# HansiZeng/scaling-retriever

Hardware: AMD Instinct MI355X
Metric: MSMARCO-Dev queries/sec end-to-end (query encode + dense brute-force top-1000) (higher is better)
Workload: dtype f32

## Files before the change

### include/sr_hip.h

```cpp
#ifndef SR_HIP_H
#define SR_HIP_H
#include <stdint.h>
#ifdef __cplusplus
extern "C" {
#endif

#define SR_OK 0
#define SR_ERR_INVALID 1
#define SR_ERR_HIP 2
#define SR_ERR_NOMEM 3
#define SR_ERR_UNSUPPORTED 4

#define SR_DTYPE_F32 0
#define SR_DTYPE_BF16 1
#define SR_DTYPE_F16 2

typedef void* sr_stream;

const char* sr_last_error(void);
int sr_version(void);
int sr_max_topk(void);

typedef struct sr_dense_index sr_dense_index;

// ... 193 lines not shown
                   sr_stream stream);
int sr_encode_rows(sr_model* m, const int64_t* d_input_ids, const int64_t* d_attention_mask, int32_t B, int32_t L,
                   const int32_t* d_row_shift, int32_t mode, int32_t fp32, float* d_out_sparse, float* d_out_dense,
                   sr_stream stream);
int sr_model_last_hidden(sr_model* m, float* d_out, int64_t capacity_rows, int64_t* n_tokens, sr_stream stream);
int sr_model_destroy(sr_model* m);

int sr_lora_merge(float* d_W, const float* d_A, const float* d_B, int64_t out_features,
                  int64_t in_features, int32_t r, float scale, sr_stream stream);

int sr_sparse_compact(const float* d_reps, int64_t B, int64_t V, int64_t* d_row_ptr,
                      int32_t* d_cols, float* d_vals, int64_t capacity, int64_t* h_nnz,
                      sr_stream stream);
int sr_sparse_compact_topm(const float* d_reps, int64_t B, int64_t V, int64_t max_terms,
                           int64_t* d_row_ptr, int32_t* d_cols, float* d_vals,
                           int64_t capacity, int64_t* h_nnz, sr_stream stream);

int sr_write_run_json(const char* path, int64_t nq, int64_t k, const float* h_scores, const int64_t* h_idx, const int32_t* h_counts,
                      const int64_t* h_qid_i64, const char* h_qid_bytes, const int64_t* h_qid_off, int64_t qid_width,
                      const int64_t* h_doc_i64, const char* h_doc_bytes, const int64_t* h_doc_off, int64_t doc_width,
                      int64_t n_docs, int32_t n_threads, int64_t* bytes_written);
int sr_write_run_json_part(const char* path, int32_t part, int64_t nq, int64_t k, const float* h_scores, const int64_t* h_idx,
                           const int32_t* h_counts, const int64_t* h_qid_i64, const char* h_qid_bytes, const int64_t* h_qid_off,
                           int64_t qid_width, const int64_t* h_doc_i64, const char* h_doc_bytes, const int64_t* h_doc_off,
                           int64_t doc_width, int64_t n_docs, int32_t n_threads, int64_t* bytes_written);
int64_t sr_run_writer_mapped_rounds(void);

int sr_gemm_bf16(const void* d_A, const void* d_W, int32_t M, int32_t N, int32_t K, int32_t epilogue,
                 void* d_C, const int32_t* d_seq_of, sr_stream stream);
int sr_gemm_f16_scaled(const void* d_A, const void* d_W, int32_t M, int32_t N, int32_t K, const float* d_a_scale,
                       const float* d_w_scale, float* d_C, sr_stream stream);
#define SR_READOUT_EMBED 0
#define SR_READOUT_LM_HEAD 1
#define SR_READOUT_NORM 2
#define SR_READOUT_ROPE_COS 3
#define SR_READOUT_ROPE_SIN 4
#define SR_READOUT_QKV 5
#define SR_READOUT_O 6
#define SR_READOUT_GATE_UP 7
#define SR_READOUT_DOWN 8
#define SR_READOUT_LN1 9
#define SR_READOUT_LN2 10
#define SR_READOUT_BIAS 11
#define SR_READOUT_F32 0
#define SR_READOUT_BF16 1
#define SR_READOUT_PLANES 2
#define SR_READOUT_W_INV 3
#define SR_READOUT_BF16_AS_F32 4
int sr_model_readout(sr_model* m, int32_t layer, int32_t buffer, int32_t kind, void* h_dst, int64_t capacity_bytes,
                     int64_t* n_bytes, int64_t* n_rows, int64_t* row_elems);
int sr_rows_split_f16(float* d_src, const float* d_embed, const int32_t* d_tok_id, const float* d_norm_w, float eps,
                      int32_t T, int32_t K, int32_t nseg, void* d_planes, float* d_a_inv, const float* d_gu_cmax,
                      float* d_act_sc, float* d_act_inv, sr_stream stream);
int sr_gu_cmax_f16(const void* d_wgu_planes, const float* d_wgu_inv, int32_t I, int32_t K, int32_t nseg, float* d_cmax,
                   sr_stream stream);
int sr_gemm_f16_planes(const void* d_A, const void* d_W, int32_t M, int32_t N, int32_t K, int32_t epilogue, int32_t a_nseg,
                       const float* d_a_scale, const float* d_w_scale, void* d_C, const int32_t* d_pos,
                       const float* d_rope_cos, const float* d_rope_sin, int32_t n_rope, int32_t head_dim,
                       const float* d_bias, const int32_t* d_seq_of, const float* d_out_scale, int32_t out_nseg,
                       sr_stream stream);
int sr_gemm_qkv_rope(const void* d_A, const void* d_W, int32_t M, int32_t N, int32_t K, void* d_C,
                     const int32_t* d_pos, const float* d_rope_cos, const float* d_rope_sin,
                     int32_t n_rope, int32_t head_dim, sr_stream stream);
int sr_gemm_qkv_rope_bias(const void* d_A, const void* d_W, int32_t M, int32_t N, int32_t K, void* d_C,
                          const int32_t* d_pos, const float* d_rope_cos, const float* d_rope_sin,
                          int32_t n_rope, int32_t head_dim, const float* d_bias, int32_t fp32_out, sr_stream stream);
int sr_attention_varlen(const void* d_qkv, void* d_out, const int32_t* d_cu_seqlens, const int32_t* d_pos,
                        const uint8_t* d_key_valid, const float* d_rope_cos, const float* d_rope_sin,
                        int32_t B, int32_t num_heads, int32_t num_kv_heads, int32_t head_dim, sr_stream stream);
int sr_attention_varlen_f32(const float* d_qkv, float* d_out_f32, void* d_out_planes, int32_t fp32_planes,
                            const int32_t* d_cu_seqlens, const uint8_t* d_key_valid, int32_t B, int32_t num_heads,
                            int32_t num_kv_heads, int32_t head_dim, int32_t max_seqlen, sr_stream stream);
int sr_rmsnorm_bf16(float* d_x, const float* d_embed, const int32_t* d_tok_id, const void* d_delta, const float* d_norm_w,
                    void* d_xn, float* d_xn_f32, float eps, int32_t T, int32_t H, sr_stream stream);
int sr_dense_head_pool(const float* d_x, const float* d_norm_w, const int32_t* d_cu_seqlens, const int32_t* d_pos,
                       const int32_t* d_pool_start, float eps, int32_t B, int32_t T, int32_t H, void* d_stats, float* d_out,
                       sr_stream stream);
int sr_sparse_finish(float* d_out, int64_t n, float scale, int32_t round_bf16, sr_stream stream);
int sr_encode_plan(const int64_t* d_input_ids, const int64_t* d_attention_mask, int32_t B, int32_t L, int32_t mode, int32_t vocab,
                   const int32_t* d_row_shift, int32_t* d_span_start, int32_t* d_span_len, int32_t* d_pool_start,
                   int32_t* d_row_len, int32_t* d_cu_seqlens, int32_t* d_tok_id, int32_t* d_pos, uint8_t* d_key_valid,
                   int32_t* d_seq_of, int64_t capacity, int64_t* n_tokens, sr_stream stream);
int sr_split_bf16(const float* d_src, int64_t n, void* d_p0, void* d_p1, void* d_p2, sr_stream stream);
int sr_topk_replay(const float* d_scores, const int64_t* d_ids, int64_t nq, int64_t n_stream, const int64_t* h_steps, int n_steps,
                   int k, int k2, int64_t select_over, int filter, int seg_n, int seg_group, float tau2_init, float pad_score,
                   float* d_out_scores, int64_t* d_out_ids, int32_t* d_out_counts, float* d_trace_tau, float* d_trace_tau2,
                   int32_t* d_trace_cand, int32_t* d_trace_run, uint64_t* d_trace_keys, sr_stream stream);

int sr_topk_collapse(const float* d_scores, const int64_t* d_ids, const int32_t* d_counts, int64_t nq, int64_t row_len, int exhaustive,
                     const int32_t* d_keys, int64_t n_keys, int k, float* d_out_scores, int64_t* d_out_ids, int32_t* d_out_keys,
                     int32_t* d_out_counts, int32_t* d_out_complete, sr_stream stream);

int sr_group_members_count(const int32_t* d_slot_keys, int64_t nq, int64_t kg, const int32_t* d_uniq_keys, int64_t n_groups,
                           const int64_t* d_member_indptr, const int64_t* d_member_ids, int64_t n_members,
                           const uint32_t* d_mask_words, int64_t n_masks, int64_t n_bits, const int32_t* d_query_group,
                           int64_t* d_out_indptr, int64_t* total, sr_stream stream);
int sr_group_members_fill(const int32_t* d_slot_keys, int64_t nq, int64_t kg, const int32_t* d_uniq_keys, int64_t n_groups,
                          const int64_t* d_member_indptr, const int64_t* d_member_ids, int64_t n_members,
                          const uint32_t* d_mask_words, int64_t n_masks, int64_t n_bits, const int32_t* d_query_group,
                          const int64_t* d_out_indptr, int64_t* d_out_ids, int64_t capacity, sr_stream stream);
int sr_segment_topm(const float* d_scores, const int64_t* d_ids, const int64_t* d_seg_indptr, int64_t n_segs, int m,
                    int use_threshold, float threshold, float pad_score, float* d_out_scores, int64_t* d_out_ids,
                    int32_t* d_out_counts, sr_stream stream);

#ifdef __cplusplus
}
#endif
#endif
```

### scaling_retriever_amd/_lib.py

```python
import contextlib
import ctypes
import os
import threading

_HERE = os.path.dirname(os.path.abspath(__file__))
LIB_PATH = os.environ.get("SR_HIP_LIB") or os.path.join(_HERE, "libsr_hip.so")

SR_OK, SR_ERR_INVALID, SR_ERR_HIP, SR_ERR_NOMEM, SR_ERR_UNSUPPORTED = 0, 1, 2, 3, 4
SR_DTYPE_F32, SR_DTYPE_BF16, SR_DTYPE_F16 = 0, 1, 2
SR_FUSE_RRF, SR_FUSE_MINMAX = 0, 1

c_void_p, c_int, c_int32, c_int64, c_float, c_char_p = (ctypes.c_void_p, ctypes.c_int, ctypes.c_int32,
                                                         ctypes.c_int64, ctypes.c_float, ctypes.c_char_p)


class SrModelConfig(ctypes.Structure):
    _fields_ = [
        ("vocab_size", c_int32), ("hidden_size", c_int32), ("intermediate_size", c_int32), ("num_layers", c_int32),
        ("num_heads", c_int32), ("num_kv_heads", c_int32), ("head_dim", c_int32),
        ("rms_norm_eps", c_float), ("rope_theta", c_float), ("rope_llama3", c_int32),
        ("rope_factor", c_float), ("rope_low_freq_factor", c_float), ("rope_high_freq_factor", c_float),
        ("rope_original_max_pos", c_int32), ("tie_word_embeddings", c_int32), ("has_lm_head", c_int32),
        ("max_batch_tokens", c_int32), ("max_batch_seqs", c_int32), ("fp32_planes", c_int32),
        ("attention_bias", c_int32),
# ... 59 lines not shown
                                         c_void_p, c_int64, c_int64, c_void_p, c_void_p, c_void_p, c_void_p]),
    "sr_sparse_range_count": (c_int, [c_void_p, c_void_p, c_void_p, c_void_p, c_int64, c_void_p, c_void_p, ctypes.POINTER(c_int64), c_void_p]),
    "sr_sparse_range_fill": (c_int, [c_void_p, c_void_p, c_void_p, c_void_p, c_int64, c_void_p, c_void_p, c_int64, c_int64, c_void_p,
                                     c_void_p, c_int64, c_void_p]),
    "sr_sparse_range_count_masked": (c_int, [c_void_p, c_void_p, c_void_p, c_void_p, c_int64, c_void_p, c_void_p, c_int64, c_void_p,
                                             ctypes.POINTER(c_int64), c_void_p]),
    "sr_sparse_range_fill_masked": (c_int, [c_void_p, c_void_p, c_void_p, c_void_p, c_int64, c_void_p, c_void_p, c_int64, c_void_p, c_int64,
                                            c_int64, c_void_p, c_void_p, c_int64, c_void_p]),
    "sr_sparse_range_count_grouped": (c_int, [c_void_p, c_void_p, c_void_p, c_void_p, c_int64, c_void_p, c_void_p, c_int64, c_int64, c_void_p,
                                              c_void_p, ctypes.POINTER(c_int64), c_void_p]),
    "sr_sparse_range_fill_grouped": (c_int, [c_void_p, c_void_p, c_void_p, c_void_p, c_int64, c_void_p, c_void_p, c_int64, c_int64, c_void_p,
                                             c_void_p, c_int64, c_int64, c_void_p, c_void_p, c_int64, c_void_p]),
    "sr_sparse_index_block_stats": (c_int, [c_void_p, ctypes.POINTER(c_int64), ctypes.POINTER(c_int64),
                                            ctypes.POINTER(c_int64)]),
    "sr_sparse_index_destroy": (c_int, [c_void_p]),
    "sr_sparse_index_cert_stats": (c_int, [c_void_p, ctypes.POINTER(c_int64)]),
    "sr_sparse_index_cert_debug": (c_int, [c_void_p, c_int, c_void_p, c_int64, c_void_p, c_int64,
                                           ctypes.POINTER(c_float), ctypes.POINTER(ctypes.c_int32)]),
    "sr_sparse_index_cert_readout": (c_int, [c_void_p, c_int, c_void_p, c_int64, ctypes.POINTER(c_int64)]),
    "sr_sparse_csr_expand_terms": (c_int, [c_void_p, c_int64, c_int64, c_void_p, c_void_p]),
    "sr_sparse_csr_build": (c_int, [c_void_p, c_void_p, c_void_p, c_int64, c_int64, c_int64, c_int, c_void_p, c_void_p,
                                    c_void_p, c_void_p]),
    "sr_topk_merge": (c_int, [c_void_p, c_void_p, c_int, c_int64, c_int, c_float, c_void_p, c_void_p, c_void_p]),
    "sr_topk_replay": (c_int, [c_void_p, c_void_p, c_int64, c_int64, c_void_p, c_int, c_int, c_int, c_int64, c_int, c_int, c_int, c_float,
                               c_float, c_void_p, c_void_p, c_void_p, c_void_p, c_void_p, c_void_p, c_void_p, c_void_p, c_void_p]),
    "sr_hybrid_union": (c_int, [c_void_p, c_void_p, c_int64, c_void_p, c_void_p, c_int64, c_void_p, c_int64, c_void_p, c_int64, c_int64,
                                c_void_p, c_void_p, c_void_p, c_void_p, c_int64, ctypes.POINTER(c_int64), c_void_p]),
    "sr_hybrid_rank": (c_int, [c_void_p, c_void_p, c_void_p, c_void_p, c_void_p, c_void_p, c_int64, c_float, c_float, c_int, c_void_p,
                               c_void_p, c_void_p, c_int64, c_int64, c_void_p, c_void_p, c_void_p, c_void_p, c_void_p, c_void_p]),
    "sr_rank_fuse": (c_int, [c_void_p, c_void_p, c_void_p, c_int, c_int64, c_int64, c_int, ctypes.POINTER(c_float), c_float, c_int, c_void_p,
                             c_void_p, c_void_p, c_void_p, c_void_p]),
    "sr_mmr_max_candidates": (c_int, []),
    "sr_dense_mmr": (c_int, [c_void_p, c_void_p, c_void_p, c_void_p, c_int64, c_int64, c_int, c_float, c_void_p, c_void_p, c_void_p, c_void_p,
                             c_void_p, c_void_p]),
    "sr_prf_max_entries": (c_int, []),
    "sr_sparse_feedback": (c_int, [c_void_p, c_void_p, c_void_p, c_int64, c_void_p, c_void_p, c_void_p, c_int64, c_int64, c_void_p, c_void_p,
                                   c_int64, c_int, c_int, c_float, c_float, c_float, c_int64, c_void_p, c_void_p, c_void_p, c_int64,
                                   ctypes.POINTER(c_int64), c_void_p]),
    "sr_dense_feedback": (c_int, [c_void_p, c_void_p, c_int64, c_void_p, c_void_p, c_int64, c_int, c_int, c_float, c_float, c_float, c_void_p,
                                  c_void_p]),
    "sr_topk_collapse": (c_int, [c_void_p, c_void_p, c_void_p, c_int64, c_int64, c_int, c_void_p, c_int64, c_int, c_void_p, c_void_p, c_void_p,
                                 c_void_p, c_void_p, c_void_p]),
    "sr_group_members_count": (c_int, [c_void_p, c_int64, c_int64, c_void_p, c_int64, c_void_p, c_void_p, c_int64, c_void_p, c_int64, c_int64,
                                       c_void_p, c_void_p, ctypes.POINTER(c_int64), c_void_p]),
    "sr_group_members_fill": (c_int, [c_void_p, c_int64, c_int64, c_void_p, c_int64, c_void_p, c_void_p, c_int64, c_void_p, c_int64, c_int64,
                                      c_void_p, c_void_p, c_void_p, c_int64, c_void_p]),
    "sr_segment_topm": (c_int, [c_void_p, c_void_p, c_void_p, c_int64, c_int, c_int, c_float, c_float, c_void_p, c_void_p, c_void_p,
                                c_void_p]),
    "sr_model_create": (c_int, [ctypes.POINTER(c_void_p), ctypes.POINTER(SrModelConfig)]),
    "sr_model_set_weight": (c_int, [c_void_p, c_char_p, c_void_p, c_int, c_int64, c_int64, c_void_p]),
    "sr_model_finalize": (c_int, [c_void_p]),
    "sr_model_readout": (c_int, [c_void_p, c_int32, c_int32, c_int32, c_void_p, c_int64, ctypes.POINTER(c_int64), ctypes.POINTER(c_int64),
                                 ctypes.POINTER(c_int64)]),
    "sr_model_weight_segments": (c_int, [c_void_p, ctypes.POINTER(ctypes.c_int32), c_int64, ctypes.POINTER(c_int64)]),
    "sr_model_fused_act_layers": (c_int, [c_void_p, ctypes.POINTER(ctypes.c_int32), c_int64, ctypes.POINTER(c_int64)]),
    "sr_encode_dense": (c_int, [c_void_p, c_void_p, c_void_p, c_int32, c_int32, c_void_p, c_void_p]),
    "sr_encode_sparse": (c_int, [c_void_p, c_void_p, c_void_p, c_int32, c_int32, c_void_p, c_void_p]),
    "sr_encode_dense_fp32": (c_int, [c_void_p, c_void_p, c_void_p, c_int32, c_int32, c_void_p, c_void_p]),
    "sr_encode_sparse_fp32": (c_int, [c_void_p, c_void_p, c_void_p, c_int32, c_int32, c_void_p, c_void_p]),
    "sr_encode_both": (c_int, [c_void_p, c_void_p, c_void_p, c_int32, c_int32, c_int32, c_void_p, c_void_p, c_void_p]),
    "sr_encode_rows": (c_int, [c_void_p, c_void_p, c_void_p, c_int32, c_int32, c_void_p, c_int32, c_int32, c_void_p, c_void_p, c_void_p]),
    "sr_model_last_hidden": (c_int, [c_void_p, c_void_p, c_int64, ctypes.POINTER(c_int64), c_void_p]),
    "sr_model_destroy": (c_int, [c_void_p]),
    "sr_lora_merge": (c_int, [c_void_p, c_void_p, c_void_p, c_int64, c_int64, c_int32, c_float, c_void_p]),
    "sr_run_writer_mapped_rounds": (c_int64, []),
    "sr_write_run_json": (c_int, [c_char_p, c_int64, c_int64, c_void_p, c_void_p, c_void_p, c_void_p, c_void_p, c_void_p, c_int64,
                                  c_void_p, c_void_p, c_void_p, c_int64, c_int64, c_int32, ctypes.POINTER(c_int64)]),
    "sr_write_run_json_part": (c_int, [c_char_p, c_int32, c_int64, c_int64, c_void_p, c_void_p, c_void_p, c_void_p, c_void_p, c_void_p, c_int64,
                                       c_void_p, c_void_p, c_void_p, c_int64, c_int64, c_int32, ctypes.POINTER(c_int64)]),
    "sr_gemm_bf16": (c_int, [c_void_p, c_void_p, c_int32, c_int32, c_int32, c_int32, c_void_p, c_void_p, c_void_p]),
    "sr_gemm_f16_scaled": (c_int, [c_void_p, c_void_p, c_int32, c_int32, c_int32, c_void_p, c_void_p, c_void_p, c_void_p]),
    "sr_rows_split_f16": (c_int, [c_void_p, c_void_p, c_void_p, c_void_p, c_float, c_int32, c_int32, c_int32, c_void_p, c_void_p, c_void_p,
                                  c_void_p, c_void_p, c_void_p]),
    "sr_gu_cmax_f16": (c_int, [c_void_p, c_void_p, c_int32, c_int32, c_int32, c_void_p, c_void_p]),
    "sr_gemm_f16_planes": (c_int, [c_void_p, c_void_p, c_int32, c_int32, c_int32, c_int32, c_int32, c_void_p, c_void_p, c_void_p, c_void_p,
                                   c_void_p, c_void_p, c_int32, c_int32, c_void_p, c_void_p, c_void_p, c_int32, c_void_p]),
    "sr_rmsnorm_bf16": (c_int, [c_void_p, c_void_p, c_void_p, c_void_p, c_void_p, c_void_p, c_void_p, c_float, c_int32, c_int32, c_void_p]),
    "sr_dense_head_pool": (c_int, [c_void_p, c_void_p, c_void_p, c_void_p, c_void_p, c_float, c_int32, c_int32, c_int32, c_void_p, c_void_p,
                                   c_void_p]),
    "sr_sparse_finish": (c_int, [c_void_p, c_int64, c_float, c_int32, c_void_p]),
    "sr_encode_plan": (c_int, [c_void_p, c_void_p, c_int32, c_int32, c_int32, c_int32, c_void_p, c_void_p, c_void_p, c_void_p, c_void_p,
                               c_void_p, c_void_p, c_void_p, c_void_p, c_void_p, c_int64, ctypes.POINTER(c_int64), c_void_p]),
    "sr_split_bf16": (c_int, [c_void_p, c_int64, c_void_p, c_void_p, c_void_p, c_void_p]),
    "sr_gemm_qkv_rope": (c_int, [c_void_p, c_void_p, c_int32, c_int32, c_int32, c_void_p, c_void_p, c_void_p, c_void_p,
                                 c_int32, c_int32, c_void_p]),
    "sr_gemm_qkv_rope_bias": (c_int, [c_void_p, c_void_p, c_int32, c_int32, c_int32, c_void_p, c_void_p, c_void_p, c_void_p,
                                      c_int32, c_int32, c_void_p, c_int32, c_void_p]),
    "sr_attention_varlen": (c_int, [c_void_p, c_void_p, c_void_p, c_void_p, c_void_p, c_void_p, c_void_p, c_int32,
                                    c_int32, c_int32, c_int32, c_void_p]),
    "sr_attention_varlen_f32": (c_int, [c_void_p, c_void_p, c_void_p, c_int32, c_void_p, c_void_p, c_int32, c_int32, c_int32,
                                        c_int32, c_int32, c_void_p]),
    "sr_sparse_compact": (c_int, [c_void_p, c_int64, c_int64, c_void_p, c_void_p, c_void_p, c_int64,
                                  ctypes.POINTER(c_int64), c_void_p]),
    "sr_sparse_compact_topm": (c_int, [c_void_p, c_int64, c_int64, c_int64, c_void_p, c_void_p, c_void_p, c_int64,
                                       ctypes.POINTER(c_int64), c_void_p]),
}

_lib = None
_lock = threading.Lock()


class SrHipError(RuntimeError):
    pass


def _bind(path):
    if not os.path.exists(path):
        raise SrHipError(
            f"{path} not found: the HIP extension is not built. There is no CPU fallback; "
            "run `make -C scaling_retriever_amd/csrc` (needs hipcc, targets gfx950).")
    import torch
    lib = ctypes.CDLL(path)
    for name, (res, args) in SIGNATURES.items():
        fn = getattr(lib, name)
        fn.restype = res
        fn.argtypes = args
    return lib


def load():
    global _lib
    with _lock:
        if _lib is None:
            _lib = _bind(LIB_PATH)
        return _lib


@contextlib.contextmanager
def library(path):
    global _lib
    other = _bind(os.path.abspath(path))
    with _lock:
        keep, _lib = _lib, other
    try:
        yield other
    finally:
        with _lock:
            _lib = keep


def check(rc, what=""):
    if rc == SR_OK:
        return
    msg = load().sr_last_error().decode("utf-8", "replace")
    if rc == SR_ERR_INVALID:
        raise ValueError(f"{what}: {msg}" if what else msg)
    if rc == SR_ERR_NOMEM:
        raise MemoryError(f"{what}: {msg}" if what else msg)
    raise SrHipError(f"{what}: [{rc}] {msg}" if what else f"[{rc}] {msg}")


def stream_ptr():
    import torch
    return ctypes.c_void_p(torch.cuda.current_stream().cuda_stream)


def require_gpu():
    import torch
    if not torch.cuda.is_available():
        raise SrHipError("no ROCm device visible: scaling_retriever_amd runs its hot path on MI355X only "
                         "(there is no CPU fallback)")
```

### scaling_retriever_amd/csrc/dense_split.h

```cpp
#pragma once
#include "common.h"
struct DenseSplitArgs {
    const unsigned short* D[3];
    const unsigned short* Q[3];
    int n_pairs;
    int pair_d[6], pair_q[6];
    int64_t row_begin, row_end;
    int H, nq;
    const float* tau;
    uint64_t* cand_keys;
    int* cand_count;
    int64_t cand_cap;
    uint32_t id_base, id_stride;
    unsigned char* seg_cnt;
    int seg_n;
    int64_t seg_off;
    int upper_bound;
    const float* dxy;
    const float* qa;
    const float* dxy_gmax;
    float sd, isd;
    int xcd_order, grid_qt, grid_dt, grid_bq, grid_bd, grid_nbq, grid_total;
    int diag;
    unsigned long long* stamps;
    const uint32_t* mask;
    const uint32_t* mask_qoff;
};
int launch_split_bf16(const float* src, unsigned short* p0, unsigned short* p1, unsigned short* p2, int64_t n_elems, hipStream_t s);
int launch_dense_split(const DenseSplitArgs& a, hipStream_t s);
int launch_dense_split_masked(const DenseSplitArgs& a, unsigned grid, size_t lds, hipStream_t s);
int launch_dense_split_grouped(const DenseSplitArgs& a, unsigned grid, size_t lds, hipStream_t s);
```

### scaling_retriever_amd/csrc/dense_split.hip

```cpp
#include "dense_split_kernel.h"

__global__ void split_bf16_kernel(const float* __restrict__ src, unsigned short* __restrict__ p0, unsigned short* __restrict__ p1,
                                  unsigned short* __restrict__ p2, int64_t n4) {
    for (int64_t i = (int64_t)blockIdx.x * blockDim.x + threadIdx.x; i < n4; i += (int64_t)gridDim.x * blockDim.x) {
        const f32x4 v = reinterpret_cast<const f32x4*>(src)[i];
        bf16x4 a, b, c;
#pragma unroll
        for (int e = 0; e < 4; ++e) {
            const unsigned short h = f32_to_bf16_sat(v[e]);
            const float r1 = v[e] - bf16_to_f32(h);
            const unsigned short m = f32_to_bf16(r1);
            const float r2 = r1 - bf16_to_f32(m);
            a[e] = (short)h;
            b[e] = (short)m;
            c[e] = (short)f32_to_bf16(r2);
        }
        reinterpret_cast<bf16x4*>(p0)[i] = a;
        if (p1) reinterpret_cast<bf16x4*>(p1)[i] = b;
        if (p2) reinterpret_cast<bf16x4*>(p2)[i] = c;
    }
}

int launch_split_bf16(const float* src, unsigned short* p0, unsigned short* p1, unsigned short* p2, int64_t n_elems, hipStream_t s) {
    const int64_t n4 = n_elems / 4;
    if (n4 == 0) return SR_OK;
    int64_t blocks = ceil_div64(n4, 256);
    if (blocks > (1 << 22)) blocks = 1 << 22;
    hipLaunchKernelGGL(split_bf16_kernel, dim3((unsigned)blocks), dim3(256), 0, s, src, p0, p1, p2, n4);
    SR_CHECK_LAUNCH();
    return SR_OK;
}

extern "C" int sr_split_bf16(const float* d_src, int64_t n, void* d_p0, void* d_p1, void* d_p2, sr_stream stream) {
    SR_REQUIRE(d_src && d_p0, "sr_split_bf16: null pointer");
    SR_REQUIRE(n >= 0 && n % 4 == 0, "sr_split_bf16: bad size n=%lld (n must be a multiple of 4)", (long long)n);
    SR_REQUIRE((uintptr_t)d_src % 16 == 0 && (uintptr_t)d_p0 % 8 == 0 && (uintptr_t)d_p1 % 8 == 0 && (uintptr_t)d_p2 % 8 == 0,
               "sr_split_bf16: d_src must be 16-byte aligned, the planes 8-byte aligned");
    return launch_split_bf16(d_src, (unsigned short*)d_p0, (unsigned short*)d_p1, (unsigned short*)d_p2, n, (hipStream_t)stream);
}

struct SplitGrid { int qt, dt, bq, bd, nbq, total; };
static inline SplitGrid split_grid(int64_t rows, int nq, int xcd_order) {
    SplitGrid g;
    g.qt = (int)ceil_div64(nq, SP_BM);
    g.dt = (int)ceil_div64(rows, SP_BN);
    g.bq = !xcd_order ? 1 : (g.qt % 4 == 0 ? 4 : g.qt % 2 == 0 ? 2 : 1);
    g.bd = 32 / g.bq;
    g.nbq = g.qt / g.bq;
    g.total = !xcd_order ? g.qt * g.dt : (int)(ceil_div64((int64_t)g.nbq * ceil_div64(g.dt, g.bd) * 32, 256) * 256);
    return g;
}

int launch_dense_split(const DenseSplitArgs& a, hipStream_t s) {
    const int64_t rows = a.row_end - a.row_begin;
    if (rows <= 0) return SR_OK;
    SR_REQUIRE(a.H % 64 == 0, "dense_split: dim %d must be a multiple of 64", a.H);
    SR_REQUIRE(a.n_pairs >= 1 && a.n_pairs <= 6 && a.n_pairs * (a.H / 64) >= 2, "dense_split: bad plane-pair count %d", a.n_pairs);
    SR_REQUIRE(!a.upper_bound || (a.n_pairs == 1 && a.dxy && a.qa), "dense_split: the upper-bound pass is one plane product");
    SR_REQUIRE(!a.mask || a.upper_bound, "dense_split: a document mask goes with the upper-bound pass only");
    SR_REQUIRE(!a.mask_qoff || a.mask, "dense_split: per-query mask offsets without a mask");
    constexpr size_t lds = 2 * (size_t)(SP_BN + SP_BM) * 128 + SP_BN * 2 * sizeof(float) + SP_BM * 4 * sizeof(float) + SP_BM * sizeof(float);
    static DeviceOnce attr_once;
    bool* attr_slot = attr_once.pending();
    if (attr_slot) {
        SR_CHECK_HIP(hipFuncSetAttribute(reinterpret_cast<const void*>(&dense_split_kernel<false, false>),
                                         hipFuncAttributeMaxDynamicSharedMemorySize, (int)lds));
        SR_CHECK_HIP(hipFuncSetAttribute(reinterpret_cast<const void*>(&dense_split_kernel<true, false>),
                                         hipFuncAttributeMaxDynamicSharedMemorySize, (int)lds));
        *attr_slot = true;
    }
    DenseSplitArgs b = a;
    if (const char* e = sr_dev_getenv("SR_SPLIT_BLOCKTEST")) if (atoi(e) == 0) b.dxy_gmax = nullptr;
    SR_REQUIRE(!b.dxy_gmax || a.row_begin % SP_BN == 0, "dense_split: the block test needs launches that start on a tile boundary");
    b.xcd_order = 1;
    if (const char* e = sr_dev_getenv("SR_SPLIT_XCD")) b.xcd_order = atoi(e);
    b.diag = 0;
#ifdef SR_DIAG_BUILD
    if (const char* e = sr_dev_getenv("SR_SPLIT_DIAG")) b.diag = atoi(e);
#endif
    b.stamps = nullptr;
#ifdef SR_DIAG_BUILD
    if (sr_dev_getenv("SR_SPLIT_STAMPS")) {
        static unsigned long long* d_st = nullptr;
        static int calls = 0;
        if (!d_st) { SR_CHECK_HIP(hipMalloc((void**)&d_st, 32)); SR_CHECK_HIP(hipMemset(d_st, 0, 32)); }
        if (++calls % 272 == 0) {
            unsigned long long h[4];
            SR_CHECK_HIP(hipMemcpy(h, d_st, 32, hipMemcpyDeviceToHost));
            if (h[3]) fprintf(stderr, "[split stamps] tiles %llu: k-loop %.2f us, epilogue issue %.2f us, drain wait %.2f us\n", h[3],
                              h[0] * 0.01 / h[3], h[1] * 0.01 / h[3], h[2] * 0.01 / h[3]);
            SR_CHECK_HIP(hipMemset(d_st, 0, 32));
        }
        b.stamps = d_st;
    }
#endif
    const SplitGrid sg = split_grid(rows, a.nq, b.xcd_order);
    b.grid_qt = sg.qt; b.grid_dt = sg.dt; b.grid_bq = sg.bq; b.grid_bd = sg.bd; b.grid_nbq = sg.nbq; b.grid_total = sg.total;
    int wgs = sr_cu_count();
    wgs -= wgs % 8;
    if (wgs < 8) wgs = 8;
    if (const char* e = sr_dev_getenv("SR_SPLIT_PERSIST")) if (atoi(e) == 0) wgs = sg.total;
    const dim3 grid((unsigned)(sg.total < wgs ? sg.total : wgs));
    if (a.mask_qoff) return launch_dense_split_grouped(b, grid.x, lds, s);
    if (a.mask) return launch_dense_split_masked(b, grid.x, lds, s);
    if (a.upper_bound) hipLaunchKernelGGL((dense_split_kernel<true, false>), grid, dim3(512), lds, s, b);
    else hipLaunchKernelGGL((dense_split_kernel<false, false>), grid, dim3(512), lds, s, b);
    SR_CHECK_LAUNCH();
    return SR_OK;
}
```

### scaling_retriever_amd/csrc/dense_split_kernel.h

```cpp
#pragma once
#include "dense_split.h"

#ifdef SR_DIAG_BUILD
#define SR_SPLIT_DIAG_BIT(a, bit) ((a).diag & (bit))
#define SR_SPLIT_STAMPS_PTR(a) ((a).stamps)
#else
#define SR_SPLIT_DIAG_BIT(a, bit) 0
#define SR_SPLIT_STAMPS_PTR(a) (static_cast<unsigned long long*>(nullptr))
#endif

typedef __bf16 mfma_bf16x8 __attribute__((ext_vector_type(8)));
typedef __attribute__((address_space(3))) void* lds_void_ptr;
typedef __attribute__((address_space(1))) const void* gbl_void_ptr;

#define SP_BN 256
#define SP_BM 256
typedef _Float16 mfma_f16x8 __attribute__((ext_vector_type(8)));
template <bool F16>
__device__ __forceinline__ f32x4 split_mma(const mfma_bf16x8& w, const mfma_bf16x8& a, const f32x4& c) {
    if constexpr (F16)
        return __builtin_amdgcn_mfma_f32_16x16x32_f16(__builtin_bit_cast(mfma_f16x8, w), __builtin_bit_cast(mfma_f16x8, a), c, 0, 0, 0);
    else
        return __builtin_amdgcn_mfma_f32_16x16x32_bf16(w, a, c, 0, 0, 0);
}
// ... 62 lines not shown
        int n = 0;
#pragma unroll
        for (int i = 0; i < NB; ++i) {
            const int lr0 = wn * NB * 16 + i * 16 + fg * 4;
            float m4 = fmaxf(fmaxf(acc[i][j][0], acc[i][j][1]), fmaxf(acc[i][j][2], acc[i][j][3]));
            if (!full) {
                m4 = -INFINITY;
#pragma unroll
                for (int r = 0; r < 4; ++r)
                    if (lr0 + r < rows_valid) m4 = fmaxf(m4, acc[i][j][r]);
            }
            if (__ballot(m4 >= line) == 0) continue;
            if constexpr (UB)
                if (pre) {
                    const float* p = xy_s + 2 * lr0;
                    const f32x4 v0 = *reinterpret_cast<const f32x4*>(p), v1 = *reinterpret_cast<const f32x4*>(p + 4);
                    const float x[4] = {v0[0], v0[2], v1[0], v1[2]}, y[4] = {v0[1], v0[3], v1[1], v1[3]};
#pragma unroll
                    for (int r = 0; r < 4; ++r)
                        acc[i][j][r] = __builtin_fmaf(qa[j][0], x[r], __builtin_fmaf(qa[j][1], y[r], acc[i][j][r]));
                }
#pragma unroll
            for (int r = 0; r < 4; ++r) {
                const float sc = acc[i][j][r];
                if constexpr (MASKED) {
                    if (lr0 + r < rows_valid && sc >= tq[j] && split_doc_allowed<true, GROUPED>(a, gid0 + (uint32_t)(lr0 + r) * a.id_stride, q)) {
                        if (seg_ok && n < SR_SEG_P) seg_dst[n] = sr_make_key(sc * out_scale[j], gid0 + (uint32_t)(lr0 + r) * a.id_stride);
                        ++n;
                    }
                } else if (lr0 + r < rows_valid && sc >= tq[j]) {
                    if (seg_ok && n < SR_SEG_P) seg_dst[n] = sr_make_key(UB ? sc * out_scale[j] : sc, gid0 + (uint32_t)(lr0 + r) * a.id_stride);
                    ++n;
                }
            }
        }
        slow[j] = n > 0 && (!seg_ok || n > SR_SEG_P);
        if (n > 0 && !slow[j]) a.seg_cnt[(int64_t)q * a.seg_n + seg_idx] = (unsigned char)n;
    }
    if (SR_SPLIT_DIAG_BIT(a, 4)) return;
    bool any_slow = false;
#pragma unroll
    for (int j = 0; j < MB; ++j) any_slow = any_slow || slow[j];
    if (__ballot(any_slow) == 0) return;
#pragma unroll
    for (int j = 0; j < MB; ++j) {
        if (__ballot(slow[j]) == 0) continue;
        const int q = q0 + wm * MB * 16 + j * 16 + frow;
        int cnt = 0;
        if (slow[j]) {
#pragma unroll
            for (int i = 0; i < NB; ++i)
#pragma unroll
                for (int r = 0; r < 4; ++r) {
                    const int lr = wn * NB * 16 + i * 16 + fg * 4 + r;
                    if constexpr (MASKED)
                        cnt += (lr < rows_valid && acc[i][j][r] >= tq[j] && split_doc_allowed<true, GROUPED>(a, gid0 + (uint32_t)lr * a.id_stride, q)) ? 1 : 0;
                    else
                    cnt += (lr < rows_valid && acc[i][j][r] >= tq[j]) ? 1 : 0;
                }
        }
        if (cnt == 0) continue;
        int p = atomicAdd(&a.cand_count[q], cnt);
        uint64_t* dst = a.cand_keys + (int64_t)q * a.cand_cap;
        const int64_t limit = a.seg_off > 0 ? a.seg_off : a.cand_cap;
#pragma unroll
        for (int i = 0; i < NB; ++i)
#pragma unroll
            for (int r = 0; r < 4; ++r) {
                const int lr = wn * NB * 16 + i * 16 + fg * 4 + r;
                const float sc = acc[i][j][r];
                if constexpr (MASKED) {
                    if (lr < rows_valid && sc >= tq[j] && split_doc_allowed<true, GROUPED>(a, gid0 + (uint32_t)lr * a.id_stride, q)) {
                        if (p < limit) dst[p] = sr_make_key(sc * out_scale[j], gid0 + (uint32_t)lr * a.id_stride);
                        ++p;
                    }
                } else if (lr < rows_valid && sc >= tq[j]) {
                    if (p < limit) dst[p] = sr_make_key(UB ? sc * out_scale[j] : sc, gid0 + (uint32_t)lr * a.id_stride);
                    ++p;
                }
            }
    }
}

__device__ __forceinline__ bool split_tile_of(const DenseSplitArgs& a, int lin, int& d_tile, int& q_tile) {
    if (!a.xcd_order) {
        q_tile = lin % a.grid_qt;
        d_tile = lin / a.grid_qt;
        return true;
    }
    const int s = lin >> 3;
    const int c = (s >> 5) * 256 + (lin & 7) * 32 + (s & 31);
    const int blk = c >> 5, w2 = c & 31;
    const int bd_i = blk / a.grid_nbq, bq_i = blk - bd_i * a.grid_nbq;
    d_tile = bd_i * a.grid_bd + w2 / a.grid_bq;
    q_tile = bq_i * a.grid_bq + w2 % a.grid_bq;
    return d_tile < a.grid_dt;
}

template <bool UB, bool MASKED, bool GROUPED = false>
__global__ __launch_bounds__(512, 2) void dense_split_kernel(DenseSplitArgs a) {
    static_assert(UB || !MASKED, "a document mask goes with the upper-bound pass only");
    static_assert(MASKED || !GROUPED, "per-query bitmaps are a kind of document mask");
    constexpr int NB = 8, MB = 4, WAVES_M = 4, HB = NB / 2;
    constexpr int W_BYTES = SP_BN * 128, STAGE_BYTES = (SP_BN + SP_BM) * 128;
    extern __shared__ __attribute__((aligned(16))) unsigned char smem[];
    float* xy_s = reinterpret_cast<float*>(smem + 2 * STAGE_BYTES);
    float* qa_s = xy_s + 2 * SP_BN;
    float* tau_s = qa_s + 4 * SP_BM;
    const int tid = threadIdx.x, lane = tid & 63, wave = tid >> 6;
    const int G = (int)gridDim.x;
    const int H = a.H;

    const int wave_s = __builtin_amdgcn_readfirstlane(wave);
    const int wn = wave_s / WAVES_M, wm = wave_s % WAVES_M;
    uint32_t doff[4], qoff[4];
    int64_t st_dbase = 0, st_qbase = 0;
    int st_pair = 0, st_k0 = 0;
    const unsigned short* st_d = a.D[a.pair_d[0]];
    const unsigned short* st_q = a.Q[a.pair_q[0]];
    int64_t st_row0 = 0;
    int st_q0 = 0;
    auto next_slot = [&](int t) {
        int d_t, q_t;
        while (t < a.grid_total && !split_tile_of(a, t, d_t, q_t)) t += G;
        return t;
    };
    auto set_tile = [&](int lin) {
        int d_tile, q_tile;
        (void)split_tile_of(a, lin, d_tile, q_tile);
        st_row0 = a.row_begin + (int64_t)d_tile * SP_BN;
        st_q0 = q_tile * SP_BM;
        st_dbase = st_row0 * H;
        st_qbase = (int64_t)st_q0 * H;
        const int64_t dleft = a.row_end - 1 - st_row0;
        const int dmax = dleft < SP_BN - 1 ? (int)dleft : SP_BN - 1, qmax = a.nq - 1 - st_q0 < SP_BM - 1 ? a.nq - 1 - st_q0 : SP_BM - 1;
        int lane_o = lane;
        asm volatile("" : "+v"(lane_o));
        const int srow = lane_o >> 3;
        const int schunk = (lane_o & 7) ^ (srow & 7);
#pragma unroll
        for (int i = 0; i < 4; ++i) {
            const int r = (wave_s * 4 + i) * 8 + srow;
            doff[i] = (uint32_t)((r < dmax ? r : dmax) * H + schunk * 8) * 2u;
            qoff[i] = (uint32_t)((r < qmax ? r : qmax) * H + schunk * 8) * 2u;
        }
        st_pair = 0; st_k0 = 0;
        st_d = a.D[a.pair_d[0]];
        st_q = a.Q[a.pair_q[0]];
    };
    auto stage_pieces = [&](int st) {
        unsigned char* wbase = smem + st * STAGE_BYTES + (wave_s * 4) * 1024;
        unsigned char* abase = smem + st * STAGE_BYTES + W_BYTES + (wave_s * 4) * 1024;
        const unsigned char* dsrc = reinterpret_cast<const unsigned char*>(st_d + (st_dbase + st_k0));
        const unsigned char* qsrc = reinterpret_cast<const unsigned char*>(st_q + (st_qbase + st_k0));
#pragma unroll
        for (int i = 0; i < 4; ++i)
            __builtin_amdgcn_global_load_lds((gbl_void_ptr)(dsrc + doff[i]), (lds_void_ptr)(wbase + i * 1024), 16, 0, 0);
#pragma unroll
        for (int i = 0; i < 4; ++i)
            __builtin_amdgcn_global_load_lds((gbl_void_ptr)(qsrc + qoff[i]), (lds_void_ptr)(abase + i * 1024), 16, 0, 0);
        st_k0 += 64;
    };
    auto stage_wrap = [&]() {
        if (st_k0 == H) {
            st_k0 = 0;
            ++st_pair;
            if (st_pair < a.n_pairs) {
                st_d = a.D[a.pair_d[st_pair]];
                st_q = a.Q[a.pair_q[st_pair]];
            }
        }
    };
    auto stage = [&](int st) {
        stage_pieces(st);
        stage_wrap();
    };

    const int frow = lane & 15, fg = lane >> 4;
    const int nkt = a.n_pairs * (H / 64);
    f32x4 acc[NB][MB];
    mfma_bf16x8 wx[HB], wy[HB], a0[MB], a1[MB];
    auto load_w = [&](int st, int kk, int h, mfma_bf16x8 (&wf)[HB]) {
        const unsigned char* wt = smem + st * STAGE_BYTES;
        const int pos = ((4 * kk + fg) ^ (frow & 7)) * 16;
#pragma unroll
        for (int i = 0; i < HB; ++i)
            wf[i] = *reinterpret_cast<const mfma_bf16x8*>(wt + (wn * NB * 16 + (h * HB + i) * 16 + frow) * 128 + pos);
    };
    auto load_a = [&](int st, int kk, mfma_bf16x8 (&af)[MB]) {
        const unsigned char* at = smem + st * STAGE_BYTES + W_BYTES;
        const int pos = ((4 * kk + fg) ^ (frow & 7)) * 16;
#pragma unroll
        for (int j = 0; j < MB; ++j)
            af[j] = *reinterpret_cast<const mfma_bf16x8*>(at + (wm * MB * 16 + j * 16 + frow) * 128 + pos);
    };
#define SR_MFMA_HALF(HH, WF, AF)                                                                              \
    _Pragma("unroll") for (int i = 0; i < HB; ++i)                                                            \
        _Pragma("unroll") for (int j = 0; j < MB; ++j)                                                        \
            acc[(HH) * HB + i][j] = split_mma<UB>(WF[i], AF[j], acc[(HH) * HB + i][j]);

    int tile = next_slot((int)blockIdx.x);
    if (tile >= a.grid_total) return;
    set_tile(tile);
    stage(0);
    stage(1);
    int buf = 0;
    bool carried = false;
    for (;;) {
        const int64_t row0 = st_row0;
        const int q0 = st_q0;
        const int tile_next = next_slot(tile + G);
        const bool has_next = tile_next < a.grid_total;
        float gx = 0.f, gy = 0.f;
        if constexpr (UB)
            if (a.dxy_gmax) {
                const float* gm = a.dxy_gmax + 2 * ((row0 >> 7) + wn);
                gx = gm[0];
                gy = gm[1];
            }
#pragma unroll
        for (int i = 0; i < NB; ++i)
#pragma unroll
            for (int j = 0; j < MB; ++j) acc[i][j] = f32x4{0.f, 0.f, 0.f, 0.f};
        if (carried) {
            asm volatile("s_waitcnt lgkmcnt(0)\n\ts_barrier" ::: "memory");
        } else {
            asm volatile("s_waitcnt vmcnt(0)" ::: "memory");
            __syncthreads();
        }
        const unsigned long long st0 = SR_SPLIT_STAMPS_PTR(a) ? __builtin_amdgcn_s_memrealtime() : 0;
        int lane_t = lane;
        asm volatile("" : "+v"(lane_t));
        if (wave_s >= 4) {
            int q = q0 + (wave_s - 4) * 64 + lane_t;
            q = q < a.nq ? q : a.nq - 1;
            __builtin_amdgcn_global_load_lds((gbl_void_ptr)(a.tau + q), (lds_void_ptr)(tau_s + (wave_s - 4) * 64), 4, 0, 0);
        }
        if constexpr (UB) {
            int64_t r = row0 + wave_s * 32 + (lane_t >> 1);
            r = r < a.row_end ? r : a.row_end - 1;
            __builtin_amdgcn_global_load_lds((gbl_void_ptr)(a.dxy + r * 2 + (lane_t & 1)), (lds_void_ptr)(xy_s + wave_s * 64), 4, 0, 0);
            if (wave_s < 4) {
                int q = q0 + wave_s * 64 + lane_t;
                q = q < a.nq ? q : a.nq - 1;
                __builtin_amdgcn_global_load_lds((gbl_void_ptr)(a.qa + (int64_t)q * 4), (lds_void_ptr)(qa_s + wave_s * 256), 16, 0, 0);
            }
        }
        if (!carried) {
            load_w(buf, 0, 0, wx);
            load_a(buf, 0, a0);
        }
        int kt = 0;
#define SR_SGB(MASK, N, ID) __builtin_amdgcn_sched_group_barrier(MASK, N, ID)
        const int n_sched = has_next ? nkt : nkt - 2;
        bool switched = false;
        while (kt < n_sched) {
        int to_go = nkt - 2 - kt;
        if (to_go <= 0) {
            if (!switched) { set_tile(tile_next); switched = true; }
            to_go = nkt - kt;
        }
        const int in_plane = (H - st_k0) >> 6;
        const int stretch = in_plane < to_go ? in_plane : to_go;
#pragma unroll 1
        for (int it = 0; it < stretch; ++it, ++kt) {
            load_w(buf, 0, 1, wy);
            load_a(buf, 1, a1);
            SR_MFMA_HALF(0, wx, a0)
#pragma unroll
            for (int i = 0; i < HB + MB; ++i) { SR_SGB(0x008, 1, 0); SR_SGB(0x100, 1, 0); }
            SR_SGB(0x008, HB * MB - HB - MB, 0);
            __builtin_amdgcn_sched_barrier(0);
            load_w(buf, 1, 0, wx);
            SR_MFMA_HALF(1, wy, a0)
#pragma unroll
            for (int i = 0; i < HB; ++i) { SR_SGB(0x008, 1, 1); SR_SGB(0x100, 1, 1); }
            SR_SGB(0x008, HB * MB - HB, 1);
            __builtin_amdgcn_sched_barrier(0);
            load_w(buf, 1, 1, wy);
            SR_MFMA_HALF(0, wx, a1)
#pragma unroll
            for (int i = 0; i < HB; ++i) { SR_SGB(0x008, 1, 2); SR_SGB(0x100, 1, 2); }
            SR_SGB(0x008, HB * MB - HB, 2);
            __builtin_amdgcn_sched_barrier(0);
            asm volatile("s_waitcnt vmcnt(0)" ::: "memory");
            __syncthreads();
            load_w(buf ^ 1, 0, 0, wx);
            load_a(buf ^ 1, 0, a0);
            stage_pieces(buf);
            SR_MFMA_HALF(1, wy, a1)
#pragma unroll
            for (int i = 0; i < HB + MB; ++i) { SR_SGB(0x008, 1, 3); SR_SGB(0x100, 1, 3); }
#pragma unroll
            for (int i = 0; i < 8; ++i) { SR_SGB(0x008, 1, 3); SR_SGB(0x010, 1, 3); }
            __builtin_amdgcn_sched_barrier(0);
            buf ^= 1;
        }
        stage_wrap();
        }
#undef SR_SGB
        for (; kt < nkt; ++kt) {
            load_w(buf, 0, 1, wy);
            SR_MFMA_HALF(0, wx, a0)
            load_w(buf, 1, 0, wx);
            load_a(buf, 1, a1);
            SR_MFMA_HALF(1, wy, a0)
            load_w(buf, 1, 1, wy);
            SR_MFMA_HALF(0, wx, a1)
            asm volatile("s_waitcnt vmcnt(0)" ::: "memory");
            __syncthreads();
            if (kt + 1 < nkt) {
                load_w(buf ^ 1, 0, 0, wx);
                load_a(buf ^ 1, 0, a0);
            }
            SR_MFMA_HALF(1, wy, a1)
            buf ^= 1;
        }
        const unsigned long long st1 = SR_SPLIT_STAMPS_PTR(a) ? __builtin_amdgcn_s_memrealtime() : 0;
        split_epilogue<UB, MASKED, GROUPED, NB, MB>(a, acc, row0, q0, wn, wm, frow, fg, xy_s, qa_s, tau_s, gx, gy);
        if (SR_SPLIT_STAMPS_PTR(a)) {
            const unsigned long long st2 = __builtin_amdgcn_s_memrealtime();
            asm volatile("s_waitcnt vmcnt(0)" ::: "memory");
            const unsigned long long st3 = __builtin_amdgcn_s_memrealtime();
            if (tid == 0) {
                atomicAdd(&a.stamps[0], st1 - st0);
                atomicAdd(&a.stamps[1], st2 - st1);
                atomicAdd(&a.stamps[2], st3 - st2);
                atomicAdd(&a.stamps[3], 1ull);
            }
        }
        if (!has_next) break;
        tile = tile_next;
        carried = true;
    }
#undef SR_MFMA_HALF
}
```

Measured before the change: 15650.

## Skip MFMA work for query strips past batch end and rotate ragged tiles

Adds a ragged mode, on by default, in which waves whose query strip lies entirely beyond nq skip the MFMA k-loop and epilogue. They still take part in the shared-memory staging and barriers so the block stays in step. It also rotates the tile slot order for the last query-block column across XCDs, so partially empty tiles do not pile up on the same dies. It remaps which wave gets which query strip so that dead strips are spread across waves, and it adds a host helper that exports the tile map. Risks include a mismatch in the barrier sequence and wave imbalance inside a block.

```diff
diff --git a/include/sr_hip.h b/include/sr_hip.h
--- a/include/sr_hip.h
+++ b/include/sr_hip.h
@@ -299,6 +299,7 @@
                    int32_t* d_row_len, int32_t* d_cu_seqlens, int32_t* d_tok_id, int32_t* d_pos, uint8_t* d_key_valid,
                    int32_t* d_seq_of, int64_t capacity, int64_t* n_tokens, sr_stream stream);
 int sr_split_bf16(const float* d_src, int64_t n, void* d_p0, void* d_p1, void* d_p2, sr_stream stream);
+int sr_dense_split_tile_map(int64_t rows, int32_t nq, int32_t* h_tiles, int64_t cap, int64_t* n_slots);
 int sr_topk_replay(const float* d_scores, const int64_t* d_ids, int64_t nq, int64_t n_stream, const int64_t* h_steps, int n_steps,
                    int k, int k2, int64_t select_over, int filter, int seg_n, int seg_group, float tau2_init, float pad_score,
                    float* d_out_scores, int64_t* d_out_ids, int32_t* d_out_counts, float* d_trace_tau, float* d_trace_tau2,
diff --git a/scaling_retriever_amd/_lib.py b/scaling_retriever_amd/_lib.py
--- a/scaling_retriever_amd/_lib.py
+++ b/scaling_retriever_amd/_lib.py
@@ -165,6 +165,7 @@
     "sr_encode_plan": (c_int, [c_void_p, c_void_p, c_int32, c_int32, c_int32, c_int32, c_void_p, c_void_p, c_void_p, c_void_p, c_void_p,
                                c_void_p, c_void_p, c_void_p, c_void_p, c_void_p, c_int64, ctypes.POINTER(c_int64), c_void_p]),
     "sr_split_bf16": (c_int, [c_void_p, c_int64, c_void_p, c_void_p, c_void_p, c_void_p]),
+    "sr_dense_split_tile_map": (c_int, [c_int64, c_int32, c_void_p, c_int64, ctypes.POINTER(c_int64)]),
     "sr_gemm_qkv_rope": (c_int, [c_void_p, c_void_p, c_int32, c_int32, c_int32, c_void_p, c_void_p, c_void_p, c_void_p,
                                  c_int32, c_int32, c_void_p]),
     "sr_gemm_qkv_rope_bias": (c_int, [c_void_p, c_void_p, c_int32, c_int32, c_int32, c_void_p, c_void_p, c_void_p, c_void_p,
diff --git a/scaling_retriever_amd/csrc/dense_split.h b/scaling_retriever_amd/csrc/dense_split.h
--- a/scaling_retriever_amd/csrc/dense_split.h
+++ b/scaling_retriever_amd/csrc/dense_split.h
@@ -21,6 +21,8 @@
     const float* dxy_gmax;
     float sd, isd;
     int xcd_order, grid_qt, grid_dt, grid_bq, grid_bd, grid_nbq, grid_total;
+    int grid_rot;
+    int ragged;
     int diag;
     unsigned long long* stamps;
     const uint32_t* mask;
diff --git a/scaling_retriever_amd/csrc/dense_split.hip b/scaling_retriever_amd/csrc/dense_split.hip
--- a/scaling_retriever_amd/csrc/dense_split.hip
+++ b/scaling_retriever_amd/csrc/dense_split.hip
@@ -39,8 +39,8 @@
     return launch_split_bf16(d_src, (unsigned short*)d_p0, (unsigned short*)d_p1, (unsigned short*)d_p2, n, (hipStream_t)stream);
 }
 
-struct SplitGrid { int qt, dt, bq, bd, nbq, total; };
-static inline SplitGrid split_grid(int64_t rows, int nq, int xcd_order) {
+struct SplitGrid { int qt, dt, bq, bd, nbq, total, rot; };
+static inline SplitGrid split_grid(int64_t rows, int nq, int xcd_order, int deal) {
     SplitGrid g;
     g.qt = (int)ceil_div64(nq, SP_BM);
     g.dt = (int)ceil_div64(rows, SP_BN);
@@ -48,7 +48,32 @@
     g.bd = 32 / g.bq;
     g.nbq = g.qt / g.bq;
     g.total = !xcd_order ? g.qt * g.dt : (int)(ceil_div64((int64_t)g.nbq * ceil_div64(g.dt, g.bd) * 32, 256) * 256);
+    const int low = g.nbq & -g.nbq;
+    g.rot = !xcd_order || !deal ? 0 : (low < 8 ? low : 8);
     return g;
+}
+static inline void split_grid_fill(DenseSplitArgs& b, const SplitGrid& sg) {
+    b.grid_qt = sg.qt; b.grid_dt = sg.dt; b.grid_bq = sg.bq; b.grid_bd = sg.bd; b.grid_nbq = sg.nbq; b.grid_total = sg.total;
+    b.grid_rot = sg.rot;
+}
+
+extern "C" int sr_dense_split_tile_map(int64_t rows, int32_t nq, int32_t* h_tiles, int64_t cap, int64_t* n_slots) {
+    SR_REQUIRE(h_tiles && n_slots, "sr_dense_split_tile_map: null pointer");
+    SR_REQUIRE(rows >= 1 && nq >= 1 && ceil_div64(rows, SP_BN) * ceil_div64(nq, SP_BM) <= (1 << 24),
+               "sr_dense_split_tile_map: bad sizes (rows=%lld nq=%d)", (long long)rows, nq);
+    DenseSplitArgs a = {};
+    a.xcd_order = 1;
+    const SplitGrid sg = split_grid(rows, nq, 1, 1);
+    split_grid_fill(a, sg);
+    SR_REQUIRE(cap >= sg.total, "sr_dense_split_tile_map: %d slots, room for %lld", sg.total, (long long)cap);
+    for (int lin = 0; lin < sg.total; ++lin) {
+        int d_tile, q_tile;
+        const bool ok = split_tile_of(a, lin, d_tile, q_tile);
+        h_tiles[2 * lin] = ok ? d_tile : -1;
+        h_tiles[2 * lin + 1] = ok ? q_tile : -1;
+    }
+    *n_slots = sg.total;
+    return SR_OK;
 }
 
 int launch_dense_split(const DenseSplitArgs& a, hipStream_t s) {
@@ -74,6 +99,8 @@
     SR_REQUIRE(!b.dxy_gmax || a.row_begin % SP_BN == 0, "dense_split: the block test needs launches that start on a tile boundary");
     b.xcd_order = 1;
     if (const char* e = sr_dev_getenv("SR_SPLIT_XCD")) b.xcd_order = atoi(e);
+    b.ragged = 1;
+    if (const char* e = sr_dev_getenv("SR_SPLIT_RAGGED")) b.ragged = atoi(e) != 0;
     b.diag = 0;
 #ifdef SR_DIAG_BUILD
     if (const char* e = sr_dev_getenv("SR_SPLIT_DIAG")) b.diag = atoi(e);
@@ -83,19 +110,22 @@
     if (sr_dev_getenv("SR_SPLIT_STAMPS")) {
         static unsigned long long* d_st = nullptr;
         static int calls = 0;
-        if (!d_st) { SR_CHECK_HIP(hipMalloc((void**)&d_st, 32)); SR_CHECK_HIP(hipMemset(d_st, 0, 32)); }
+        if (!d_st) { SR_CHECK_HIP(hipMalloc((void**)&d_st, 64)); SR_CHECK_HIP(hipMemset(d_st, 0, 64)); }
         if (++calls % 272 == 0) {
-            unsigned long long h[4];
-            SR_CHECK_HIP(hipMemcpy(h, d_st, 32, hipMemcpyDeviceToHost));
+            unsigned long long h[8];
+            SR_CHECK_HIP(hipMemcpy(h, d_st, 64, hipMemcpyDeviceToHost));
             if (h[3]) fprintf(stderr, "[split stamps] tiles %llu: k-loop %.2f us, epilogue issue %.2f us, drain wait %.2f us\n", h[3],
                               h[0] * 0.01 / h[3], h[1] * 0.01 / h[3], h[2] * 0.01 / h[3]);
-            SR_CHECK_HIP(hipMemset(d_st, 0, 32));
+            if (h[5] && h[3] > h[5])
+                fprintf(stderr, "[split stamps] k-loop of the %llu tiles of a query tile that ends beyond the batch %.2f us, of the others %.2f us\n",
+                        h[5], h[4] * 0.01 / h[5], (h[0] - h[4]) * 0.01 / (h[3] - h[5]));
+            SR_CHECK_HIP(hipMemset(d_st, 0, 64));
         }
         b.stamps = d_st;
     }
 #endif
-    const SplitGrid sg = split_grid(rows, a.nq, b.xcd_order);
-    b.grid_qt = sg.qt; b.grid_dt = sg.dt; b.grid_bq = sg.bq; b.grid_bd = sg.bd; b.grid_nbq = sg.nbq; b.grid_total = sg.total;
+    const SplitGrid sg = split_grid(rows, a.nq, b.xcd_order, b.ragged);
+    split_grid_fill(b, sg);
     int wgs = sr_cu_count();
     wgs -= wgs % 8;
     if (wgs < 8) wgs = 8;
diff --git a/scaling_retriever_amd/csrc/dense_split_kernel.h b/scaling_retriever_amd/csrc/dense_split_kernel.h
--- a/scaling_retriever_amd/csrc/dense_split_kernel.h
+++ b/scaling_retriever_amd/csrc/dense_split_kernel.h
@@ -168,7 +168,7 @@
     }
 }
 
-__device__ __forceinline__ bool split_tile_of(const DenseSplitArgs& a, int lin, int& d_tile, int& q_tile) {
+__host__ __device__ __forceinline__ bool split_tile_of(const DenseSplitArgs& a, int lin, int& d_tile, int& q_tile) {
     if (!a.xcd_order) {
         q_tile = lin % a.grid_qt;
         d_tile = lin / a.grid_qt;
@@ -176,8 +176,10 @@
     }
     const int s = lin >> 3;
     const int c = (s >> 5) * 256 + (lin & 7) * 32 + (s & 31);
-    const int blk = c >> 5, w2 = c & 31;
+    const int blk = c >> 5;
+    int w2 = c & 31;
     const int bd_i = blk / a.grid_nbq, bq_i = blk - bd_i * a.grid_nbq;
+    if (bq_i == a.grid_nbq - 1) w2 = (w2 + ((bd_i * a.grid_rot) >> 3)) & 31;
     d_tile = bd_i * a.grid_bd + w2 / a.grid_bq;
     q_tile = bq_i * a.grid_bq + w2 % a.grid_bq;
     return d_tile < a.grid_dt;
@@ -198,7 +200,8 @@
     const int H = a.H;
 
     const int wave_s = __builtin_amdgcn_readfirstlane(wave);
-    const int wn = wave_s / WAVES_M, wm = wave_s % WAVES_M;
+    const int wn = wave_s / WAVES_M, wm = (a.ragged ? wave_s + 2 * wn : wave_s) % WAVES_M;
+    auto strip_live = [&](int q0) { return !a.ragged || q0 + wm * (MB * 16) < a.nq; };
     uint32_t doff[4], qoff[4];
     int64_t st_dbase = 0, st_qbase = 0;
     int st_pair = 0, st_k0 = 0;
@@ -295,6 +298,7 @@
     for (;;) {
         const int64_t row0 = st_row0;
         const int q0 = st_q0;
+        const bool live = strip_live(q0);
         const int tile_next = next_slot(tile + G);
         const bool has_next = tile_next < a.grid_total;
         float gx = 0.f, gy = 0.f;
@@ -348,6 +352,15 @@
         }
         const int in_plane = (H - st_k0) >> 6;
         const int stretch = in_plane < to_go ? in_plane : to_go;
+        if (!live) {
+#pragma unroll 1
+            for (int it = 0; it < stretch; ++it, ++kt) {
+                asm volatile("s_waitcnt vmcnt(0)" ::: "memory");
+                __syncthreads();
+                stage_pieces(buf);
+                buf ^= 1;
+            }
+        } else
 #pragma unroll 1
         for (int it = 0; it < stretch; ++it, ++kt) {
             load_w(buf, 0, 1, wy);
@@ -385,6 +398,16 @@
         stage_wrap();
         }
 #undef SR_SGB
+        if (!live && has_next && strip_live(st_q0)) {
+            load_w(buf, 0, 0, wx);
+            load_a(buf, 0, a0);
+        }
+        if (!live)
+            for (; kt < nkt; ++kt) {
+                asm volatile("s_waitcnt vmcnt(0)" ::: "memory");
+                __syncthreads();
+                buf ^= 1;
+            }
         for (; kt < nkt; ++kt) {
             load_w(buf, 0, 1, wy);
             SR_MFMA_HALF(0, wx, a0)
@@ -403,7 +426,7 @@
             buf ^= 1;
         }
         const unsigned long long st1 = SR_SPLIT_STAMPS_PTR(a) ? __builtin_amdgcn_s_memrealtime() : 0;
-        split_epilogue<UB, MASKED, GROUPED, NB, MB>(a, acc, row0, q0, wn, wm, frow, fg, xy_s, qa_s, tau_s, gx, gy);
+        if (live) split_epilogue<UB, MASKED, GROUPED, NB, MB>(a, acc, row0, q0, wn, wm, frow, fg, xy_s, qa_s, tau_s, gx, gy);
         if (SR_SPLIT_STAMPS_PTR(a)) {
             const unsigned long long st2 = __builtin_amdgcn_s_memrealtime();
             asm volatile("s_waitcnt vmcnt(0)" ::: "memory");
@@ -413,6 +436,10 @@
                 atomicAdd(&a.stamps[1], st2 - st1);
                 atomicAdd(&a.stamps[2], st3 - st2);
                 atomicAdd(&a.stamps[3], 1ull);
+                if (q0 + SP_BM > a.nq) {
+                    atomicAdd(&a.stamps[4], st1 - st0);
+                    atomicAdd(&a.stamps[5], 1ull);
+                }
             }
         }
         if (!has_next) break;
```

Result: no change. 15680 (median of 6 runs) (+0.2%).
